# mees/hulc2

Hardware: AMD Instinct MI355X
Metric: play-sequences/sec/node (seq_len=32, 200x200 RGB) (higher is better)
Workload: dtype bf16; 1 GPU; BASELINE configs[1]: synthetic CALVIN-shaped batch, Hulc2.training_step fwd+bwd+allreduce+Adam, static CNN 200x200 + gripper CNN 84x84, lang = random (B,384) embeddings, dropout 0.1, gripper_control on; sequences_per_gpu_step=64, seq_len=32, parallelism=dp1, launch=hipGraph replay (fwd+bwd graph, all-reduce, optimizer graph), frames=fp32 NCHW, already transformed (the reference's dataloader output), gradient_allreduce=none (one rank, no process group), exact_forward_sites=encfc,goal,head,txl

## Files before the change

hulc2_amd/csrc/conv_wgrad_band.hip:

```cpp
#include "hulc_common.h"
#include "hulc_abi_internal.h"
#include "u8_frames.h"
#include <stdlib.h>

namespace {

struct WBandP {
    const void* X; const void* dY;
    int x_dtype, dy_dtype;
    int Nimg, H, W, OH, OW, R, F;
    long x_sn, x_sy, x_sx, x_sc;
    long dy_sn, dy_sy, dy_sx;
    float* partial_w;
    float* partial_b;
    int u8, pad; const int* shift; const int* fidx;
};

template <int C, int CT, int TH, int TW, int S, bool NCHW, int XCH, int YCH, int BPC, bool PURE16, bool STAMP = false>
__global__ __launch_bounds__(512, 2 * BPC) void conv_wgrad_band_kernel(WBandP p, unsigned long long* stamps = nullptr) {
    constexpr int NT = 512;
    constexpr int COUT = CT * 32;
    constexpr int K = TH * TW * C, KTN = K / 32;
    constexpr int MAXT = (KTN + 7) / 8;
    constexpr int PS = NCHW ? 2 : C * 2 + 16;
    extern __shared__ __attribute__((aligned(16))) char smem[];

    const int tid = threadIdx.x, lane = tid & 63, wave = tid >> 6;
    const int r = lane & 31, h = lane >> 5;
    const int Wb = p.W;
    const int Wp = Wb;
    const int bands = (p.OH + p.R - 1) / p.R;
    const float inv_OW = fast_rcp(p.OW);
    const int nunits = p.F > 1 ? (p.Nimg + p.F - 1) / p.F : p.Nimg * bands;
    const int rows_max = (p.F - 1) * p.H + (p.R - 1) * S + TH;
    const int npix_max = (p.F * p.R * p.OW + 15) / 16 * 16;
    constexpr bool TR = !NCHW && PURE16;
    constexpr int DROW = COUT * 2 + 16;
    const int AT_ROW = TR ? 0 : npix_max * 2 + 16;
    char* xband = smem;
    const int PP = (rows_max * Wp + 7) / 8 * 8;
    const int xbytes = NCHW ? C * PP * 2 : rows_max * Wb * PS;
    char* at = smem + (xbytes + 15) / 16 * 16;
    int* pixoff = (int*)(at + (TR ? npix_max * DROW : COUT * AT_ROW));

    constexpr bool SPLIT18 = KTN == 18 && CT == 2;
    int koff[MAXT]; bool kt_live[MAXT];
    int kts[MAXT];
    bool ct_live[MAXT][CT];
#pragma unroll
    for (int t = 0; t < MAXT; ++t) {
        int kt = wave + 8 * t;
        if (SPLIT18) kt = t < 2 ? 2 * wave + t : 16 + (wave >> 1);
        kts[t] = kt;
        kt_live[t] = SPLIT18 ? (t < 2 || wave < 4) : kt < KTN;
#pragma unroll
        for (int i = 0; i < CT; ++i) ct_live[t][i] = kt_live[t] && (!SPLIT18 || t < 2 || i == (wave & 1));
        const int k = (kt_live[t] ? kt : 0) * 32 + r;
        if (NCHW) { const int c = k / (TH * TW), kh = (k / TW) % TH, kw = k % TW; koff[t] = (c * PP + kh * Wp + kw) * 2; }
// ... 77 lines not shown
            const int qc = inb ? q : 0;
            const long off = (long)n * p.dy_sn + (long)r0 * p.dy_sy + (long)qc * p.dy_sx + ycc * 8;
            uint4 v;
            const float keep = inb ? 1.f : 0.f;
            if (PURE16 || p.dy_dtype == HULC_BF16) {
                v = *(const uint4*)((const uint16_t*)p.dY + off);
            } else {
                const float4* qq = (const float4*)((const float*)p.dY + off);
                const float4 a = qq[0], b = qq[1];
                v.x = pack_bf16x2(a.x, a.y); v.y = pack_bf16x2(a.z, a.w); v.z = pack_bf16x2(b.x, b.y); v.w = pack_bf16x2(b.z, b.w);
                bsum[0] += keep * a.x; bsum[1] += keep * a.y; bsum[2] += keep * a.z; bsum[3] += keep * a.w;
                bsum[4] += keep * b.x; bsum[5] += keep * b.y; bsum[6] += keep * b.z; bsum[7] += keep * b.w;
            }
            ypre[j] = v;
        }
    };
    int po_R = -1, po_npix = -1;
    auto stage_store = [&](int unit) {
        int n, r0, R, rows, npix; unit_geom(unit, n, r0, R, rows, npix);
        if (NCHW) {
            const int nflt = rows * p.W, items = (nflt + 7) / 8;
#pragma unroll
            for (int j = 0; j < XCH; ++j) {
                const int c = j / (XCH / C), id = tid + (j % (XCH / C)) * NT;
                if (id < items) *(uint4*)(xband + (c * PP + id * 8) * 2) = xpre[j];
            }
        } else {
            const int npx = rows * Wb, cc = tid % XCPP;
#pragma unroll
            for (int j = 0; j < XCH; ++j) {
                const int px = tid / XCPP + j * (NT / XCPP);
                if (px < npx) *(uint4*)(xband + px * PS + cc * 16) = xpre[j];
            }
        }
        const int npad = (npix + 15) / 16 * 16, ycc = tid % YCPP;
#pragma unroll
        for (int j = 0; j < YCH; ++j) {
            const int q = tid / YCPP + j * (NT / YCPP);
            if (q < npad) {
                const bool inb = q < npix;
                const uint32_t w[4] = {inb ? ypre[j].x : 0u, inb ? ypre[j].y : 0u, inb ? ypre[j].z : 0u, inb ? ypre[j].w : 0u};
                if (PURE16 || p.dy_dtype == HULC_BF16) {
#pragma unroll
                    for (int e = 0; e < 4; ++e) { bsum[2 * e] += __uint_as_float(w[e] << 16); bsum[2 * e + 1] += __uint_as_float(w[e] & 0xffff0000u); }
                }
                if (TR) *(uint4*)(at + q * DROW + ycc * 16) = make_uint4(w[0], w[1], w[2], w[3]);
                else
#pragma unroll
                for (int e = 0; e < 8; ++e) {
                    const uint16_t bits = (uint16_t)((e & 1) ? (w[e >> 1] >> 16) : (w[e >> 1] & 0xffffu));
                    *(uint16_t*)(at + (ycc * 8 + e) * AT_ROW + q * 2) = bits;
                }
            }
        }
        if (R != po_R || npix != po_npix)
        for (int q = tid; q < npad; q += NT) {
            const int qc = q < npix ? q : npix - 1;
            const int ppf = R * p.OW, f = fast_div(qc, fast_rcp(ppf)), qq = qc - f * ppf;
            const int oy = fast_div(qq, inv_OW), ox = qq - oy * p.OW;
            pixoff[q] = NCHW ? ((oy * S) * Wp + ox * S) * 2 : ((f * p.H + oy * S) * Wb + ox * S) * PS;
        }
        po_R = R; po_npix = npix;
    };

    int unit = blockIdx.x;
    if (unit < nunits) { stage_load(unit); stage_store(unit); }
    __syncthreads();
    unsigned long long t_ph[6] = {0, 0, 0, 0, 0, 0}, t_units = 0, c0 = 0, c1 = 0, c2 = 0, c3 = 0, c4 = 0, c5 = 0;
    for (; unit < nunits; unit += gridDim.x) {
        const int next = unit + gridDim.x;
        if (STAMP) c0 = __builtin_readcyclecounter();
        const bool pre = next < nunits, stagger = TR;
        int n, r0, R, rows, npix; unit_geom(unit, n, r0, R, rows, npix);
        const int nsteps = (npix + 15) / 16;
        const int bat = stagger ? ((wave * nsteps) >> 3) & ~1 : 0;
        if (pre && !stagger) stage_load(next);
        if (STAMP) c1 = __builtin_readcyclecounter();

        if (TR) {
            typedef short v4s __attribute__((ext_vector_type(4)));
// ... 90 lines not shown
            for (int t = 0; t < MAXT; ++t) {
                if (!kt_live[t]) continue;
                union { uint32_t w[4]; bf16x8_t b; } x;
#pragma unroll
                for (int e = 0; e < 4; ++e) {
                    const uint32_t lo = *(const uint16_t*)(xband + po[2 * e] + koff[t]);
                    const uint32_t hi = *(const uint16_t*)(xband + po[2 * e + 1] + koff[t]);
                    x.w[e] = lo | (hi << 16);
                }
#pragma unroll
                for (int i = 0; i < CT; ++i)
                    if (ct_live[t][i]) acc[t][i] = __builtin_amdgcn_mfma_f32_32x32x16_bf16(a[i], x.b, acc[t][i], 0, 0, 0);
            }
        }
        if (STAMP) c2 = __builtin_readcyclecounter();
        __syncthreads();
        if (STAMP) { c3 = __builtin_readcyclecounter(); asm volatile("s_waitcnt vmcnt(0)" ::: "memory"); c4 = __builtin_readcyclecounter(); }
        if (next < nunits) stage_store(next);
        if (STAMP) c5 = __builtin_readcyclecounter();
        __syncthreads();
        if (STAMP) {
            const unsigned long long c6 = __builtin_readcyclecounter();
            t_ph[0] += c1 - c0; t_ph[1] += c2 - c1; t_ph[2] += c3 - c2; t_ph[3] += c4 - c3; t_ph[4] += c5 - c4; t_ph[5] += c6 - c5; t_units += 1;
        }
    }
    if (STAMP && stamps && lane == 0) {
        unsigned long long* o = stamps + ((long)blockIdx.x * 8 + wave) * 7;
#pragma unroll
        for (int e = 0; e < 6; ++e) o[e] = t_ph[e];
        o[6] = t_units;
// ... 401 lines not shown
        static bool stamp_attr = false;
        if (!stamp_attr) {
            if (hipFuncSetAttribute((const void*)conv1_wgrad_kernel<XCH, YCH, false, true>, hipFuncAttributeMaxDynamicSharedMemorySize, 80 * 1024) != hipSuccess) return -2;
            stamp_attr = true;
        }
        conv1_wgrad_kernel<XCH, YCH, false, true><<<grid, 512, (size_t)lds_of(R), s>>>(p, (unsigned long long*)strtoull(se, nullptr, 0));
    } else
    if (p.u8) conv1_wgrad_kernel<XCH, YCH, true><<<grid, 512, (size_t)lds_of(R), s>>>(p);
    else conv1_wgrad_kernel<XCH, YCH, false><<<grid, 512, (size_t)lds_of(R), s>>>(p);
    const long Rw = 32L * K;
    const int nbw = (int)((Rw + 63) / 64);
    wband_reduce_kernel<<<nbw + (db ? 1 : 0), 1024, 0, s>>>(p.partial_w, dw, grid, Rw, accumulate, 0, 64, nbw, p.partial_b, db, 32);
    return 0;
}

template <int C, int CT, int TH, int TW, int S, bool NCHW, int XCH, int YCH, int BPC, bool PURE16 = false>
int launch_wband(WBandP& p, float* dw, float* db, void* ws, long ws_bytes, int dw_oihw, int accumulate, hipStream_t s) {
    constexpr int COUT = CT * 32, K = TH * TW * C;
    constexpr int PS = NCHW ? 2 : C * 2 + 16;
    const int Wb = p.W, Wp = Wb;
    if (NCHW && p.W % 4) return -1;
    static_assert(!NCHW || XCH % C == 0, "NCHW staging: XCH items split evenly over the channel planes");
    auto lds_of = [&](int R, int F) -> long {
        const int rows = (F - 1) * p.H + (R - 1) * S + TH;
        const long xb = NCHW ? (long)C * (((long)rows * Wp + 7) / 8 * 8) * 2 : (long)rows * Wb * PS;
        const long npad = ((long)F * R * p.OW + 15) / 16 * 16;
        const long dyb = (!NCHW && PURE16) ? npad * (COUT * 2 + 16) : (long)COUT * (npad * 2 + 16);
        return (xb + 15) / 16 * 16 + dyb + npad * 4 + 64;
    };
    auto fits = [&](int R, int F) -> bool {
        const int rows = (F - 1) * p.H + (R - 1) * S + TH;
        const long xitems = NCHW ? ((long)rows * p.W + 7) / 8 * C : (long)rows * Wb * (C / 8);
        const long yitems = (((long)F * R * p.OW + 15) / 16 * 16) * (COUT / 8);
        return lds_of(R, F) <= (160 * 1024 - 256) / BPC && xitems <= (long)XCH * 512 && yitems <= (long)YCH * 512;
    };
    int R = p.OH, F = 1;
    while (R > 1 && !fits(R, 1)) --R;
    if (!fits(R, 1)) return -1;
    int nunits;
    if (R == p.OH && !NCHW) {
        while (F < p.Nimg && fits(R, F + 1)) ++F;
        nunits = (p.Nimg + F - 1) / F;
    } else {
        const int bands = (p.OH + R - 1) / R;
        R = (p.OH + bands - 1) / bands;
        nunits = p.Nimg * bands;
    }
    if ((long)F * R * p.OW < 96) return -1;
    p.R = R; p.F = F;
    const int slots = 256 * BPC;
    const int per = (nunits + slots - 1) / slots;
    const int grid = (nunits + per - 1) / per;
    if ((long)grid * COUT * (K + 1) * 4 > ws_bytes) return -1;
    p.partial_w = (float*)ws;
    p.partial_b = db ? p.partial_w + (long)grid * COUT * K : nullptr;
    auto kern = conv_wgrad_band_kernel<C, CT, TH, TW, S, NCHW, XCH, YCH, BPC, PURE16>;
    static bool attr_set = false;
    if (!attr_set) {
        if (hipFuncSetAttribute((const void*)kern, hipFuncAttributeMaxDynamicSharedMemorySize, 160 * 1024) != hipSuccess) return -2;
        attr_set = true;
    }
    const char* se = getenv("HULC_WB_STAMPS");
    if (se && *se && PURE16 && !NCHW) {
        auto kst = conv_wgrad_band_kernel<C, CT, TH, TW, S, NCHW, XCH, YCH, BPC, PURE16, true>;
        static bool st_attr = false;
        if (!st_attr) {
            if (hipFuncSetAttribute((const void*)kst, hipFuncAttributeMaxDynamicSharedMemorySize, 160 * 1024) != hipSuccess) return -2;
            st_attr = true;
        }
        kst<<<grid, 512, (size_t)lds_of(R, F), s>>>(p, (unsigned long long*)strtoull(se, nullptr, 0));
    } else
    kern<<<grid, 512, (size_t)lds_of(R, F), s>>>(p, nullptr);
    const long Rw = (long)COUT * K;
    const int nbw = (int)((Rw + 63) / 64);
    wband_reduce_kernel<<<nbw + (db ? 1 : 0), 1024, 0, s>>>(p.partial_w, dw, grid, Rw, accumulate, (dw_oihw && !NCHW) ? C : 0, TH * TW, nbw, p.partial_b, db,
                                                          COUT);
    return 0;
}
// ... 33 lines not shown
            q.xs = (const void* const*)x_slot; q.xs2 = (const void* const*)x2_slot;
            if ((x_slot || x2_slot) && (u8 || !x_slot || (x2_slot && !x2) || ((uintptr_t)x_slot | (uintptr_t)x2_slot) % 8))
                return hulc_fail(-6, "conv1 weight gradient: frame slots are for fp32 frames (x_slot with every launch, x2_slot next to x2), 8-byte aligned");
            if (x2) {
                q.X2 = u8 ? (const float*)((const unsigned char*)x2 - (long)n_split * 3 * H * W) : (const float*)x2 - (long)n_split * 3 * H * W;
                q.nsplit = n_split;
            }
            rc = launch_conv1_wgrad(q, dw, db, ws, ws_bytes, accumulate, s);
        }
    }
    else return (x2 || x_slot) ? hulc_fail(-6, "conv weight gradient: x2 / frame slots are for conv1 only") : 1;
    if (rc == -1) return 1;
    if (rc < 0) return hulc_fail(-8, "conv wgrad band: could not raise the dynamic LDS limit");
    return 0;
}
```

hulc2_amd/csrc/pointwise.hip:

```cpp
#include "hulc_common.h"
#include "hulc_abi_internal.h"
#include <stdlib.h>

namespace {

__global__ __launch_bounds__(256) void spatial_softmax_fwd_kernel(const void* __restrict__ x, int x_dtype, int N, int HW, int C,
                                                                  const float* __restrict__ xmap, const float* __restrict__ ymap,
                                                                  const float* __restrict__ temperature, float* __restrict__ out,
                                                                  float* __restrict__ stats) {
    __shared__ float red[4][4][64];
    const int lane = threadIdx.x & 63, wave = threadIdx.x >> 6;
    const int n = blockIdx.x;
    const bool act = lane < C;
    const float invT = 1.0f / temperature[0];
    const long base = (long)n * HW * C + lane;
    const int per = (HW + 3) / 4, p0 = wave * per, p1 = p0 + per < HW ? p0 + per : HW;
    float m = -INFINITY;
    if (act)
        for (int p = p0; p < p1; ++p) m = fmaxf(m, load_elem(x, x_dtype, base + (long)p * C) * invT);
    red[wave][0][lane] = m;
    __syncthreads();
    m = fmaxf(fmaxf(red[0][0][lane], red[1][0][lane]), fmaxf(red[2][0][lane], red[3][0][lane]));
    float s = 0.f, sx = 0.f, sy = 0.f;
    if (act)
// ... 162 lines not shown
}
__global__ __launch_bounds__(256) void spatial_softmax_bwd64_kernel(const void* __restrict__ x, int x_dtype, int HW,
                                                                    const float* __restrict__ xmap, const float* __restrict__ ymap,
                                                                    const float* __restrict__ temperature, const float* __restrict__ out,
                                                                    const float* __restrict__ stats, const float* __restrict__ dout,
                                                                    void* __restrict__ dx, int dx_dtype, int relu_mask) {
    const int lane = threadIdx.x & 63, wave = threadIdx.x >> 6;
    const int cg = lane & 7, pl = lane >> 3;
    const int n = blockIdx.x;
    const float invT = 1.0f / temperature[0];
    const long base = (long)n * HW * 64 + cg * 8;
    float m[8], k[8], ex[8], ey[8], gx[8], gy[8];
#pragma unroll
    for (int j = 0; j < 8; ++j) {
        const int c = cg * 8 + j;
        m[j] = stats[((long)n * 64 + c) * 2]; k[j] = invT / stats[((long)n * 64 + c) * 2 + 1];
        ex[j] = out[(long)n * 128 + 2 * c]; ey[j] = out[(long)n * 128 + 2 * c + 1];
        gx[j] = dout[(long)n * 128 + 2 * c]; gy[j] = dout[(long)n * 128 + 2 * c + 1];
    }
    for (int p = wave * 8 + pl; p < HW; p += 32) {
        Chunk8 c; chunk_load_contig(c, x, x_dtype, base + (long)p * 64);
        const float xm = xmap[p], ym = ymap[p];
        float g[8];
#pragma unroll
        for (int j = 0; j < 8; ++j) {
            g[j] = k[j] * __expf(c.v[j] * invT - m[j]) * (gx[j] * (xm - ex[j]) + gy[j] * (ym - ey[j]));
            if (relu_mask && !(c.v[j] > 0.f)) g[j] = 0.f;
        }
        const long o = base + (long)p * 64;
        if (dx_dtype == HULC_BF16) *(uint4*)((uint16_t*)dx + o) = make_uint4(pack_bf16x2(g[0], g[1]), pack_bf16x2(g[2], g[3]), pack_bf16x2(g[4], g[5]), pack_bf16x2(g[6], g[7]));
        else { ((float4*)((float*)dx + o))[0] = make_float4(g[0], g[1], g[2], g[3]); ((float4*)((float*)dx + o))[1] = make_float4(g[4], g[5], g[6], g[7]); }
    }
}


__global__ __launch_bounds__(256) void layernorm_fwd_kernel(const float* __restrict__ x, const float* __restrict__ o, float drop_p,
                                                            unsigned long long seed, const unsigned long long* __restrict__ seed_dev,
                                                            const float* __restrict__ gamma,
                                                            const float* __restrict__ beta, float eps, int R, int D,
                                                            float* __restrict__ pre_out, float* __restrict__ y,
                                                            float* __restrict__ mean_out, float* __restrict__ rstd_out,
                                                            int n_o = 1, long o_stride = 0, long ld_y = 0) {
    const int lane = threadIdx.x & 63;
// ... 649 lines not shown
```

hulc2_amd/functional.py:

```python
from typing import List, Optional, Sequence, Tuple

import os

import torch

from . import gradsink
from . import kernels as kn
from .shadow import weight_operand


def _scoped(cls):
    fwd, bwd = cls.forward, cls.backward

    def forward(ctx, *args):
        ctx._compute = kn.backward_compute()
        return fwd(ctx, *args)

    def backward(ctx, *grads):
        if ctx._compute == kn.get_compute():
            return bwd(ctx, *grads)
        with kn.compute_scope(ctx._compute):
            return bwd(ctx, *grads)

    forward.__doc__, backward.__doc__ = fwd.__doc__, bwd.__doc__
# ... 329 lines not shown
    def forward(ctx, grad_premasked, aug, w1, b1, w2, b2, w3, b3, *xs):
        xs = [_c(x) for x in xs]
        pad, shifts, indices = (aug if aug is not None else (0, [None] * len(xs), [None] * len(xs)))
        Ns = [x.shape[0] if ix is None else ix.numel() for x, ix in zip(xs, indices)]
        N = sum(Ns)
        u8 = xs[0].dtype == torch.uint8
        if u8:
            _, H, W, C = xs[0].shape
        else:
            _, C, H, W = xs[0].shape
        ws, bs = (w1, w2, w3), (b1, b2, b3)
        acts, dims = [], []
        inp, h, w_, cin = None, H, W, C
        want_bits = _act_dtype() == torch.bfloat16 and any(ctx.needs_input_grad[2:8])
        bits = [None, None, None]
        exact_out = False
        if isinstance(grad_premasked, tuple):
            grad_premasked, exact_out = grad_premasked
        a3_exact = _act_dtype() == torch.bfloat16 and kn.base_mode() == "bf16" and (exact_out or "a3" in kn.fp32_sites())
        for li, (k, s) in enumerate(ConvStackFn.GEOM):
            cout = ws[li].shape[0]
            nchw = li == 0
            w2d = weight_operand(ws[li], "oihw_flat" if nchw else "ohwi")
            oh, ow = kn.conv_out_hw(h, w_, k, k, s)
            twin = a3_exact and li == 2
            f16_twin = twin and (h, w_, cin, cout, k, s) == (23, 23, 64, 64, 3, 1)
            y = torch.empty(N, oh, ow, cout, dtype=(torch.float16 if f16_twin else torch.float32) if twin else _act_dtype(), device=xs[0].device)
            y16 = torch.empty(N, oh, ow, cout, dtype=torch.bfloat16, device=xs[0].device) if twin else None
            if want_bits and li < 2 and cout % 32 == 0 and (li > 0 or cout == 32):
                bits[li] = torch.empty(N * oh * ow * (cout // 32), dtype=torch.int32, device=xs[0].device)
            if li == 0:
                off = 0
                w_lo = weight_operand(ws[0], "oihw_flat_lo") if (not u8 and _act_dtype() == torch.bfloat16 and kn.base_mode() == "bf16"
# ... 24 lines not shown
                        raise
                    y = torch.empty(N, oh, ow, cout, dtype=torch.float32, device=xs[0].device)
                    kn.conv2d_fwd(inp, w2d, bs[li], y, N, h, w_, cin, cout, k, k, s, nchw, relu=True, relu_bits=bits[li], y_bf16=y16)
            dims.append((h, w_, cin, cout, k, s, nchw))
            acts.append(y16 if y16 is not None else y)
            inp, h, w_, cin = y, oh, ow, cout
        a3_f32 = y if (a3_exact and y16 is not None) else None
        saved = acts
        if kn.backward_compute() == "bf16" and acts[0].dtype != torch.bfloat16:
            saved = []
            for a in acts:
                h = torch.empty(a.shape, dtype=torch.bfloat16, device=a.device)
                kn.cast_f32_to_bf16(a, h, a.numel())
                saved.append(h)
        ctx.g_dtype = saved[1].dtype
        ctx.save_for_backward(saved[0], saved[1], saved[2], w2, w3, *xs)
        ctx.conv_w, ctx.conv_b = ws, bs
        ctx.relu_bits = bits
        ctx.aug = (pad, shifts, indices)
        ctx.meta = (dims, grad_premasked, Ns)
        if a3_f32 is not None:
            ctx.mark_non_differentiable(a3_f32)
            ctx.set_materialize_grads(False)
            return acts[2], a3_f32
        return acts[2]

    @staticmethod
    def backward(ctx, da3, *unused):
        a1, a2, a3, w2, w3, *xs = ctx.saved_tensors
        dims, premasked, Ns = ctx.meta
        if da3 is None:
            da3 = torch.zeros_like(a3)
        N = sum(Ns)
        g = _c(da3)
        if premasked and g.dtype != ctx.g_dtype:
            h = torch.empty(g.shape, dtype=ctx.g_dtype, device=g.device)
            kn.cast_f32_to_bf16(g, h, g.numel())
            g = h
        if not premasked:
            gz = torch.empty(g.shape, dtype=torch.float32, device=g.device)
            kn.relu_bwd(g.float() if g.dtype != torch.float32 else g, a3, gz, g.numel())
            g = gz
        inputs = (None, a1, a2)
        weights = (None, w2, w3)
        grads_w, grads_b = [None] * 3, [None] * 3
# ... 13 lines not shown
                paired = False
                if _conv1_pair_ok(xs, xs[0].dtype == torch.uint8, None, cout, shifts, indices) and g.dtype == torch.bfloat16:
                    pair_shift, pair_index = getattr(ctx, "pair_aug", (None, None))
                    try:
                        kn.conv2d_bwd_weight(xs[0], g, dw, db, N, h, w_, cin, cout, k, k, s, nchw, dw_oihw=True, accumulate=acc,
                                             x2=None if pair_index is not None else xs[1], aug_shift=pair_shift, aug_pad=pad, frame_index=pair_index)
                        paired = True
                    except kn._L.HulcKernelError as e:
                        if not _pair_not_covered(e):
                            raise
                if not paired:
                    for j, (x, n, sh, ix) in enumerate(zip(xs, Ns, shifts, indices)):
                        kn.conv2d_bwd_weight(x, g[off:off + n], dw, db, n, h, w_, cin, cout, k, k, s, nchw, dw_oihw=True, accumulate=acc or j > 0,
                                             aug_shift=sh, aug_pad=pad, frame_index=ix)
                        off += n
            else:
                kn.conv2d_bwd_weight(inputs[li], g, dw, db, N, h, w_, cin, cout, k, k, s, nchw, dw_oihw=True, accumulate=acc)
            grads_w[li] = None if sunk else dw.view(cout, cin, k, k)
            grads_b[li] = None if sunk else db
            if li > 0:
                inp = inputs[li]
                wt = weight_operand(weights[li], "ihwo")
                dx = torch.empty(N, h, w_, cin, dtype=inp.dtype, device=g.device)
                kn.conv2d_bwd_data(g, wt, dx, inp, N, h, w_, cin, cout, k, k, s, relu_bits=ctx.relu_bits[li - 1])
                g = dx
        return (None, None, grads_w[0], grads_b[0], grads_w[1], grads_b[1], grads_w[2], grads_b[2], *([None] * len(xs)))


def conv_stack(x, params, grad_premasked=False, aug_pad=0, aug_shifts=None, frame_index=None, exact_out=False):
    xs = list(x) if isinstance(x, (list, tuple)) else [x]
    aug = None
    if xs[0].dtype == torch.uint8:
        sh = list(aug_shifts) if isinstance(aug_shifts, (list, tuple)) else [aug_shifts] * len(xs)
        ix = list(frame_index) if isinstance(frame_index, (list, tuple)) else [frame_index] * len(xs)
        aug = (int(aug_pad), [None if t is None else _c(t.reshape(-1, 2).to(torch.int32)) for t in sh],
               [None if t is None else _c(t.reshape(-1).to(torch.int32)) for t in ix])
    out = ConvStackFn.apply((bool(grad_premasked), True) if exact_out else grad_premasked, aug, *params, *xs)
    if isinstance(out, tuple):
        out[0]._hulc_f32 = out[1]
        return out[0]
    return out


def exact_map(a: torch.Tensor):
    t = getattr(a, "_hulc_f32", None)
    return t if (t is not None and t.shape == a.shape) else None


@_scoped
class SpatialSoftmaxFn(torch.autograd.Function):

    @staticmethod
    def forward(ctx, a, xmap, ymap, temperature, a_exact=None):
        N, H, W, C = a.shape
        out = _f32(N, 2 * C, like=a)
# ... 909 lines not shown
```

hulc2_amd/kernels.py:

```python
import ctypes

import torch

from . import lib as _L

F32, BF16, F16 = 0, 1, 2
_COMPUTE = {"bf16": BF16, "fp32": F32, "f32": F32}
_compute_mode = BF16


_base_mode = "bf16"
_bwd_mode = None


def set_compute(mode: str) -> None:
    global _compute_mode, _base_mode, _bwd_mode
    if mode not in ("bf16", "fp32", "mixed"):
        raise ValueError(mode)
    _base_mode, _bwd_mode = mode, None
    _compute_mode = _COMPUTE["bf16" if mode == "mixed" else mode]


def get_compute() -> str:
    return "bf16" if _compute_mode == BF16 else "fp32"
# ... 440 lines not shown
                      aug_shift=None, aug_pad=0, frame_index=None, x2=None):
    _require_cuda(x, dy, dw, db)
    _require_contiguous(x=x, dy=dy, dw=dw)
    d = _conv_desc(N, H, W, Cin, Cout, KH, KW, stride, x_nchw, F32 if x.dtype == torch.uint8 else _dt(x), _dt(dy), F32, False, compute)
    d.dw_oihw, d.dw_accumulate = int(dw_oihw), int(accumulate)
    _u8_frames(d, x, aug_shift, aug_pad, frame_index)
    _second_frames(d, x, x2, N, Cin, H, W)
    if compute is None and frame_index is None and dy.dtype == torch.bfloat16:
        _slot_fields(d, x, x2, H, W, Cin, Cout, KH, stride, x_nchw)
    nbytes = _L.load().hulc_conv2d_bwd_weight_workspace(ctypes.byref(d))
    ws = torch.empty(nbytes // 4, dtype=torch.float32, device=x.device)
    oh, ow = conv_out_hw(H, W, KH, KW, stride)
    macs = float(N) * oh * ow * Cout * Cin * KH * KW
    _call("hulc_conv2d_bwd_weight", ctypes.byref(d), x, dy, dw, db, ws, key=("conv2d_bwd_weight", N, H, W, Cin, Cout, KH, stride), flops=2 * macs,
          nbytes=_nbytes(x, dy, dw, db) + (_nbytes(x2) if x2 is not None else 0))
    return dw, db


_c = ctypes


def _call(name, *args, key=None, flops=0.0, nbytes=0.0):
    lib = _L.load()
    conv = []
    for a in args:
        if isinstance(a, torch.Tensor):
            _require_cuda(a)
            a = a.data_ptr()
        conv.append(a)
    with _Timed(key or (name,), flops, nbytes):
# ... 970 lines not shown
```

hulc2_amd/models/perceptual_encoders/vision_network.py:

```python
from typing import Optional, Tuple

import torch
import torch.nn as nn

from hulc2_amd import functional as HF
from hulc2_amd import kernels as kn


class SpatialSoftmax(nn.Module):

    def __init__(self, num_rows: int, num_cols: int, temperature: Optional[float] = None):
        super().__init__()
        self.num_rows, self.num_cols = num_rows, num_cols
        a = torch.linspace(-1.0, 1.0, num_cols).reshape(-1, 1).expand(num_cols, num_rows)
        b = torch.linspace(-1.0, 1.0, num_rows).reshape(1, -1).expand(num_cols, num_rows)
        self.register_buffer("x_map", a.reshape(-1).clone())
        self.register_buffer("y_map", b.reshape(-1).clone())
        if temperature:
            self.register_buffer("temperature", torch.ones(1) * temperature)
        else:
            self.temperature = nn.Parameter(torch.ones(1))
        self.coords = None

    def forward(self, a_nhwc: torch.Tensor) -> torch.Tensor:
        if isinstance(self.temperature, nn.Parameter) and self.temperature.requires_grad:
            raise NotImplementedError("learnable spatial-softmax temperature is not on the configured path "
                                      "(conf/model/perceptual_encoder/rgb_static/default.yaml: spatial_softmax_temp 1.0)")
        out = HF.spatial_softmax(a_nhwc, self.x_map, self.y_map, self.temperature)
        self.coords = out.detach()
        return out


class VisionNetwork(nn.Module):
    def __init__(self, input_width: int, input_height: int, activation_function: str, dropout_vis_fc: float,
                 l2_normalize_output: bool, visual_features: int, num_c: int, use_sinusoid: bool,
                 spatial_softmax_temp: float):
        super().__init__()
        if activation_function != "ReLU" or use_sinusoid or l2_normalize_output or dropout_vis_fc != 0.0:
            raise NotImplementedError("hulc2_amd VisionNetwork implements the configured path only: ReLU, no sinusoid, "
                                      "no l2-normalise, dropout_vis_fc 0 (conf/model/perceptual_encoder/rgb_static/default.yaml)")
        self.act_fn = nn.ReLU()
        w, h = input_width, input_height
        for k, s in ((8, 4), (4, 2), (3, 1)):
# ... 2 lines not shown
        self.spatial_softmax = SpatialSoftmax(num_rows=w, num_cols=h, temperature=temp)
        self.conv_model = nn.Sequential(nn.Conv2d(num_c, 32, 8, stride=4), self.act_fn, nn.Conv2d(32, 64, 4, stride=2),
                                        self.act_fn, nn.Conv2d(64, 64, 3, stride=1), self.act_fn)
        self.fc1 = nn.Sequential(nn.Linear(128, 512), self.act_fn, nn.Dropout(dropout_vis_fc))
        self.fc2 = nn.Linear(512, visual_features)
        self.ln = nn.LayerNorm(visual_features)

    def lo_operands(self):
        return [(self.fc1[0].weight, "lo"), (self.fc2.weight, "lo"), (self.conv_model[0].weight, "oihw_flat_lo")]

    def conv_params(self):
        c = self.conv_model
        return (c[0].weight, c[0].bias, c[2].weight, c[2].bias, c[4].weight, c[4].bias)

    def forward(self, x: torch.Tensor, aug_shift=None, aug_pad: int = 0, frame_index=None, pre_ln: bool = False) -> torch.Tensor:
        a3 = HF.conv_stack(x, self.conv_params(), grad_premasked=True, aug_pad=aug_pad, aug_shifts=aug_shift, frame_index=frame_index)
        feat = self.spatial_softmax(a3)
        with kn.site_scope("encfc"):
            y = HF.mlp2_rows(feat, self.fc1[0].weight, self.fc1[0].bias, self.fc2.weight, self.fc2.bias)
        if pre_ln:
            return y
        return HF.layer_norm(y, self.ln.weight, self.ln.bias, self.ln.eps)

    @staticmethod
    def calc_out_size(w: int, h: int, kernel_size: int, padding: int, stride: int) -> Tuple[int, int]:
        return (w - kernel_size + 2 * padding) // stride + 1, (h - kernel_size + 2 * padding) // stride + 1
```

include/hulc2_amd.h:

```cpp
#ifndef HULC2_AMD_H
#define HULC2_AMD_H

#ifdef __cplusplus
extern "C" {
#endif

#define HULC_F32 0
#define HULC_BF16 1
#define HULC_F16 2

const char* hulc_last_error(void);
int hulc_abi_version(void);
int hulc_set_coop_share(int n);
int hulc_stream_create(void** out);

typedef struct {
    const void* A; const void* B; void* C;
    const float* bias; const void* add; const void* mask;
    int M, N, K;
    long lda, ldb, ldc, ld_add, ld_mask;
    int a_dtype, b_dtype, c_dtype, add_dtype, mask_dtype;
    int a_kmajor, b_kmajor;
    int relu, accumulate;
    float alpha, mask_scale, drop_p;
// ... 18 lines not shown
    int aug_pad;
    const int* aug_shift;
    const int* frame_index;
    void* relu_bits;
    const void* w_lo;
    const void* x2;
    int n_split;
    const void* x_slot;
    const void* x2_slot;
    void* y_bf16;
} hulc_conv_desc;
int hulc_conv2d_fwd(const hulc_conv_desc* d, const void* x, const void* w, const float* bias, void* y, void* stream);
int hulc_conv2d_bwd_data(const hulc_conv_desc* d, const void* dy, const void* wt, void* dx, const void* relu_src, void* stream);
long hulc_conv2d_bwd_weight_workspace(const hulc_conv_desc* d);
int hulc_conv2d_bwd_weight(const hulc_conv_desc* d, const void* x, const void* dy, float* dw, float* db, void* ws, void* stream);

int hulc_spatial_softmax_fwd(const void* x, int x_dtype, int N, int HW, int C, const float* xmap, const float* ymap,
                             const float* temperature, float* out, float* stats, void* stream);
int hulc_spatial_softmax_bwd(const void* x, int x_dtype, int N, int HW, int C, const float* xmap, const float* ymap,
                             const float* temperature, const float* out, const float* stats, const float* dout,
                             void* dx, int dx_dtype, int relu_mask, void* stream);
int hulc_layernorm_fwd(const float* x, const float* o, float drop_p, unsigned long long seed, const unsigned long long* seed_dev,
                       const float* gamma, const float* beta, float eps, int R, int D, float* pre_out, float* y, float* mean,
                       float* rstd, void* stream);
int hulc_layernorm_slab_fwd(const float* x, const float* o, int n_o, long o_stride, float drop_p, unsigned long long seed,
                            const unsigned long long* seed_dev, const float* gamma, const float* beta, float eps, int R, int D,
                            float* pre_out, float* y, float* mean, float* rstd, void* stream);
int hulc_layernorm_fwd_ld(const float* x, const float* gamma, const float* beta, float eps, int R, int D, float* y, long ld_y, float* mean,
                          float* rstd, void* stream);
int hulc_layernorm_bwd_ld(const float* dy, long ld_dy, const float* pre, const float* mean, const float* rstd, const float* gamma, int R, int D,
// ... 261 lines not shown
```

Measured before the change: 21030 play-sequences/s.

## Fuse spatial-softmax backward into conv3 weight-gradient band kernel

Moves the spatial-softmax forward inside the conv stack autograd function. Its backward, which turns a3 plus the softmax stats into dA3, now runs in the staging phase of the 64->64 conv3 weight-gradient band kernel. The kernel computes dA3 per tile in registers, writes it out for the later data-gradient pass, and uses it straight away for dW/db. This removes a separate pointwise kernel and one read of dA3 from memory, at the cost of extra LDS for the coordinate maps and stats, extra waitcnt syncs, and a geometry-specific path with a fallback.

```diff
diff --git a/hulc2_amd/csrc/conv_wgrad_band.hip b/hulc2_amd/csrc/conv_wgrad_band.hip
--- a/hulc2_amd/csrc/conv_wgrad_band.hip
+++ b/hulc2_amd/csrc/conv_wgrad_band.hip
@@ -1,6 +1,7 @@
 #include "hulc_common.h"
 #include "hulc_abi_internal.h"
 #include "u8_frames.h"
+#include "spatial_softmax.h"
 #include <stdlib.h>
 
 namespace {
@@ -14,9 +15,12 @@
     float* partial_w;
     float* partial_b;
     int u8, pad; const int* shift; const int* fidx;
+    const float* xmap; const float* ymap; const float* temperature;
+    const float* ss_out; const float* ss_stats; const float* ss_dout;
+    void* dy_out;
 };
 
-template <int C, int CT, int TH, int TW, int S, bool NCHW, int XCH, int YCH, int BPC, bool PURE16, bool STAMP = false>
+template <int C, int CT, int TH, int TW, int S, bool NCHW, int XCH, int YCH, int BPC, bool PURE16, bool STAMP = false, bool SSM = false>
 __global__ __launch_bounds__(512, 2 * BPC) void conv_wgrad_band_kernel(WBandP p, unsigned long long* stamps = nullptr) {
     constexpr int NT = 512;
     constexpr int COUT = CT * 32;
@@ -42,6 +46,12 @@
     const int xbytes = NCHW ? C * PP * 2 : rows_max * Wb * PS;
     char* at = smem + (xbytes + 15) / 16 * 16;
     int* pixoff = (int*)(at + (TR ? npix_max * DROW : COUT * AT_ROW));
+    static_assert(!SSM || (TR && COUT == 64), "the fused spatial-softmax backward is built for the bf16 64-channel NHWC instance");
+    constexpr int SSM_HWP = 448;
+    float* const ssc = (float*)(pixoff + npix_max);
+    float* const smx = ssc + 384;
+    float* const smy = smx + SSM_HWP;
+    const float ss_invT = SSM ? 1.0f / p.temperature[0] : 1.f;
 
     constexpr bool SPLIT18 = KTN == 18 && CT == 2;
     int koff[MAXT]; bool kt_live[MAXT];
@@ -149,6 +159,14 @@
             }
             ypre[j] = v;
         }
+        if (SSM && wave == 0) {
+            const long so = (long)n * 128 + (lane & 31) * 4;
+            __builtin_amdgcn_global_load_lds((const void __attribute__((address_space(1)))*)((lane < 32 ? p.ss_stats : p.ss_out) + so),
+                                             (void __attribute__((address_space(3)))*)ssc, 16, 0, 0);
+            if (lane < 32)
+                __builtin_amdgcn_global_load_lds((const void __attribute__((address_space(1)))*)(p.ss_dout + so),
+                                                 (void __attribute__((address_space(3)))*)(ssc + 256), 16, 0, 0);
+        }
     };
     int po_R = -1, po_npix = -1;
     auto stage_store = [&](int unit) {
@@ -169,12 +187,42 @@
             }
         }
         const int npad = (npix + 15) / 16 * 16, ycc = tid % YCPP;
+        if (SSM) {
+            uint32_t yw[YCH][4];
+            float xm[YCH], ym[YCH];
+#pragma unroll
+            for (int j = 0; j < YCH; ++j) {
+                const int q = tid / YCPP + j * (NT / YCPP);
+                const int pos = r0 * p.OW + (q < npix ? q : 0);
+                xm[j] = smx[pos]; ym[j] = smy[pos];
+                yw[j][0] = ypre[j].x; yw[j][1] = ypre[j].y; yw[j][2] = ypre[j].z; yw[j][3] = ypre[j].w;
+            }
+#pragma unroll
+            for (int e = 0; e < 4; ++e) {
+                const float4 st = *(const float4*)(ssc + ycc * 16 + 4 * e), eo = *(const float4*)(ssc + 128 + ycc * 16 + 4 * e),
+                             go = *(const float4*)(ssc + 256 + ycc * 16 + 4 * e);
+                const float k0 = hulc_ssm::bwd_scale(ss_invT, st.y), k1 = hulc_ssm::bwd_scale(ss_invT, st.w);
+#pragma unroll
+                for (int j = 0; j < YCH; ++j) {
+                    const float a0 = __uint_as_float(yw[j][e] << 16), a1 = __uint_as_float(yw[j][e] & 0xffff0000u);
+                    yw[j][e] = pack_bf16x2(hulc_ssm::bwd_elem(a0, ss_invT, st.x, k0, go.x, go.y, eo.x, eo.y, xm[j], ym[j], true),
+                                           hulc_ssm::bwd_elem(a1, ss_invT, st.z, k1, go.z, go.w, eo.z, eo.w, xm[j], ym[j], true));
+                    asm volatile("" : "+v"(yw[j][e]));
+                }
+            }
+#pragma unroll
+            for (int j = 0; j < YCH; ++j) ypre[j] = make_uint4(yw[j][0], yw[j][1], yw[j][2], yw[j][3]);
+        }
 #pragma unroll
         for (int j = 0; j < YCH; ++j) {
             const int q = tid / YCPP + j * (NT / YCPP);
             if (q < npad) {
                 const bool inb = q < npix;
                 const uint32_t w[4] = {inb ? ypre[j].x : 0u, inb ? ypre[j].y : 0u, inb ? ypre[j].z : 0u, inb ? ypre[j].w : 0u};
+                if (SSM) {
+                    if (inb)
+                        *(uint4*)((uint16_t*)p.dy_out + ((long)n * p.dy_sn + (long)r0 * p.dy_sy + (long)q * p.dy_sx + ycc * 8)) = make_uint4(w[0], w[1], w[2], w[3]);
+                }
                 if (PURE16 || p.dy_dtype == HULC_BF16) {
 #pragma unroll
                     for (int e = 0; e < 4; ++e) { bsum[2 * e] += __uint_as_float(w[e] << 16); bsum[2 * e + 1] += __uint_as_float(w[e] & 0xffff0000u); }
@@ -199,6 +247,13 @@
     };
 
     int unit = blockIdx.x;
+    if (SSM) {
+        for (int i = tid; i < p.OH * p.OW; i += NT) { smx[i] = p.xmap[i]; smy[i] = p.ymap[i]; }
+        if (unit < nunits) stage_load(unit);
+        __builtin_amdgcn_s_waitcnt(0x0F70);
+        __syncthreads();
+        if (unit < nunits) stage_store(unit);
+    } else
     if (unit < nunits) { stage_load(unit); stage_store(unit); }
     __syncthreads();
     unsigned long long t_ph[6] = {0, 0, 0, 0, 0, 0}, t_units = 0, c0 = 0, c1 = 0, c2 = 0, c3 = 0, c4 = 0, c5 = 0;
@@ -319,6 +374,7 @@
             }
         }
         if (STAMP) c2 = __builtin_readcyclecounter();
+        if (SSM && wave == 0) __builtin_amdgcn_s_waitcnt(0x0F70);
         __syncthreads();
         if (STAMP) { c3 = __builtin_readcyclecounter(); asm volatile("s_waitcnt vmcnt(0)" ::: "memory"); c4 = __builtin_readcyclecounter(); }
         if (next < nunits) stage_store(next);
@@ -750,7 +806,7 @@
     return 0;
 }
 
-template <int C, int CT, int TH, int TW, int S, bool NCHW, int XCH, int YCH, int BPC, bool PURE16 = false>
+template <int C, int CT, int TH, int TW, int S, bool NCHW, int XCH, int YCH, int BPC, bool PURE16 = false, bool SSM = false>
 int launch_wband(WBandP& p, float* dw, float* db, void* ws, long ws_bytes, int dw_oihw, int accumulate, hipStream_t s) {
     constexpr int COUT = CT * 32, K = TH * TW * C;
     constexpr int PS = NCHW ? 2 : C * 2 + 16;
@@ -762,7 +818,7 @@
         const long xb = NCHW ? (long)C * (((long)rows * Wp + 7) / 8 * 8) * 2 : (long)rows * Wb * PS;
         const long npad = ((long)F * R * p.OW + 15) / 16 * 16;
         const long dyb = (!NCHW && PURE16) ? npad * (COUT * 2 + 16) : (long)COUT * (npad * 2 + 16);
-        return (xb + 15) / 16 * 16 + dyb + npad * 4 + 64;
+        return (xb + 15) / 16 * 16 + dyb + npad * 4 + 64 + (SSM ? (384 + 2 * 448) * 4 : 0);
     };
     auto fits = [&](int R, int F) -> bool {
         const int rows = (F - 1) * p.H + (R - 1) * S + TH;
@@ -783,6 +839,7 @@
         nunits = p.Nimg * bands;
     }
     if ((long)F * R * p.OW < 96) return -1;
+    if (SSM && (F != 1 || p.OH * p.OW > 448)) return -1;
     p.R = R; p.F = F;
     const int slots = 256 * BPC;
     const int per = (nunits + slots - 1) / slots;
@@ -790,14 +847,14 @@
     if ((long)grid * COUT * (K + 1) * 4 > ws_bytes) return -1;
     p.partial_w = (float*)ws;
     p.partial_b = db ? p.partial_w + (long)grid * COUT * K : nullptr;
-    auto kern = conv_wgrad_band_kernel<C, CT, TH, TW, S, NCHW, XCH, YCH, BPC, PURE16>;
+    auto kern = conv_wgrad_band_kernel<C, CT, TH, TW, S, NCHW, XCH, YCH, BPC, PURE16, false, SSM>;
     static bool attr_set = false;
     if (!attr_set) {
         if (hipFuncSetAttribute((const void*)kern, hipFuncAttributeMaxDynamicSharedMemorySize, 160 * 1024) != hipSuccess) return -2;
         attr_set = true;
     }
     const char* se = getenv("HULC_WB_STAMPS");
-    if (se && *se && PURE16 && !NCHW) {
+    if (se && *se && PURE16 && !NCHW && !SSM) {
         auto kst = conv_wgrad_band_kernel<C, CT, TH, TW, S, NCHW, XCH, YCH, BPC, PURE16, true>;
         static bool st_attr = false;
         if (!st_attr) {
@@ -861,3 +918,30 @@
     if (rc < 0) return hulc_fail(-8, "conv wgrad band: could not raise the dynamic LDS limit");
     return 0;
 }
+
+extern "C" int hulc_conv2d_bwd_weight_ssm(const hulc_conv_desc* d, const void* x, const void* a3, const float* xmap, const float* ymap,
+                                          const float* temperature, const float* out, const float* stats, const float* dout, void* dy_out,
+                                          float* dw, float* db, void* ws, void* stream) {
+    if (!d || !x || !a3 || !xmap || !ymap || !temperature || !out || !stats || !dout || !dy_out || !dw || !ws)
+        return hulc_fail(-1, "hulc_conv2d_bwd_weight_ssm: null pointer");
+    if (d->N <= 0 || d->x_nchw || d->Cin != 64 || d->Cout != 64 || d->KH != 3 || d->KW != 3 || d->stride != 1 || d->H != 23 || d->W != 23)
+        return hulc_fail(-2, "hulc_conv2d_bwd_weight_ssm: covers the 64 -> 64 channel 3 x 3 stride-1 layer on 23 x 23 NHWC frames only");
+    if (d->x_dtype != HULC_BF16 || d->y_dtype != HULC_BF16 || d->compute != HULC_BF16)
+        return hulc_fail(-6, "hulc_conv2d_bwd_weight_ssm: bf16 maps and bf16 compute only");
+    if (d->x2 || d->x_slot || d->x2_slot || d->x_u8_nhwc || d->frame_index || d->aug_shift)
+        return hulc_fail(-6, "hulc_conv2d_bwd_weight_ssm: a second frame tensor, frame slots and uint8 frames belong to conv1");
+    if (((uintptr_t)x | (uintptr_t)a3 | (uintptr_t)dy_out | (uintptr_t)out | (uintptr_t)stats | (uintptr_t)dout) % 16)
+        return hulc_fail(-4, "hulc_conv2d_bwd_weight_ssm: x, a3, dy_out, out, stats and dout are 16-byte aligned");
+    WBandP p;
+    p.u8 = 0; p.pad = 0; p.shift = nullptr; p.fidx = nullptr;
+    p.X = x; p.dY = a3; p.x_dtype = HULC_BF16; p.dy_dtype = HULC_BF16;
+    p.Nimg = d->N; p.H = 23; p.W = 23; p.OH = 21; p.OW = 21; p.R = 1; p.F = 1;
+    p.x_sn = 23L * 23 * 64; p.x_sy = 23L * 64; p.x_sx = 64; p.x_sc = 1;
+    p.dy_sn = 21L * 21 * 64; p.dy_sy = 21L * 64; p.dy_sx = 64;
+    p.xmap = xmap; p.ymap = ymap; p.temperature = temperature; p.ss_out = out; p.ss_stats = stats; p.ss_dout = dout; p.dy_out = dy_out;
+    const int rc = launch_wband<64, 2, 3, 3, 1, false, 5, 4, 1, true, true>(p, dw, db, ws, hulc_conv2d_bwd_weight_workspace(d), d->dw_oihw, d->dw_accumulate,
+                                                                           (hipStream_t)stream);
+    if (rc == -1) return hulc_fail(-6, "hulc_conv2d_bwd_weight_ssm: the band plan does not fit (LDS or workspace)");
+    if (rc < 0) return hulc_fail(-8, "conv wgrad band: could not raise the dynamic LDS limit");
+    return hulc_check_launch("hulc_conv2d_bwd_weight_ssm");
+}
diff --git a/hulc2_amd/csrc/pointwise.hip b/hulc2_amd/csrc/pointwise.hip
--- a/hulc2_amd/csrc/pointwise.hip
+++ b/hulc2_amd/csrc/pointwise.hip
@@ -1,5 +1,6 @@
 #include "hulc_common.h"
 #include "hulc_abi_internal.h"
+#include "spatial_softmax.h"
 #include <stdlib.h>
 
 namespace {
@@ -200,7 +201,7 @@
 #pragma unroll
     for (int j = 0; j < 8; ++j) {
         const int c = cg * 8 + j;
-        m[j] = stats[((long)n * 64 + c) * 2]; k[j] = invT / stats[((long)n * 64 + c) * 2 + 1];
+        m[j] = stats[((long)n * 64 + c) * 2]; k[j] = hulc_ssm::bwd_scale(invT, stats[((long)n * 64 + c) * 2 + 1]);
         ex[j] = out[(long)n * 128 + 2 * c]; ey[j] = out[(long)n * 128 + 2 * c + 1];
         gx[j] = dout[(long)n * 128 + 2 * c]; gy[j] = dout[(long)n * 128 + 2 * c + 1];
     }
@@ -209,10 +210,7 @@
         const float xm = xmap[p], ym = ymap[p];
         float g[8];
 #pragma unroll
-        for (int j = 0; j < 8; ++j) {
-            g[j] = k[j] * __expf(c.v[j] * invT - m[j]) * (gx[j] * (xm - ex[j]) + gy[j] * (ym - ey[j]));
-            if (relu_mask && !(c.v[j] > 0.f)) g[j] = 0.f;
-        }
+        for (int j = 0; j < 8; ++j) g[j] = hulc_ssm::bwd_elem(c.v[j], invT, m[j], k[j], gx[j], gy[j], ex[j], ey[j], xm, ym, relu_mask != 0);
         const long o = base + (long)p * 64;
         if (dx_dtype == HULC_BF16) *(uint4*)((uint16_t*)dx + o) = make_uint4(pack_bf16x2(g[0], g[1]), pack_bf16x2(g[2], g[3]), pack_bf16x2(g[4], g[5]), pack_bf16x2(g[6], g[7]));
         else { ((float4*)((float*)dx + o))[0] = make_float4(g[0], g[1], g[2], g[3]); ((float4*)((float*)dx + o))[1] = make_float4(g[4], g[5], g[6], g[7]); }
diff --git a/hulc2_amd/csrc/spatial_softmax.h b/hulc2_amd/csrc/spatial_softmax.h
--- /dev/null
+++ b/hulc2_amd/csrc/spatial_softmax.h
@@ -0,0 +1,14 @@
+#pragma once
+#include "hulc_common.h"
+
+namespace hulc_ssm {
+
+HULC_DEVICE float bwd_scale(float invT, float sum) { return invT / sum; }
+
+HULC_DEVICE float bwd_elem(float x, float invT, float m, float k, float gx, float gy, float ex, float ey, float xm, float ym, bool relu_mask) {
+    float g = k * __expf(x * invT - m) * (gx * (xm - ex) + gy * (ym - ey));
+    if (relu_mask && !(x > 0.f)) g = 0.f;
+    return g;
+}
+
+}
diff --git a/hulc2_amd/functional.py b/hulc2_amd/functional.py
--- a/hulc2_amd/functional.py
+++ b/hulc2_amd/functional.py
@@ -367,9 +367,9 @@
         inp, h, w_, cin = None, H, W, C
         want_bits = _act_dtype() == torch.bfloat16 and any(ctx.needs_input_grad[2:8])
         bits = [None, None, None]
-        exact_out = False
+        exact_out, ssm = False, None
         if isinstance(grad_premasked, tuple):
-            grad_premasked, exact_out = grad_premasked
+            grad_premasked, exact_out, ssm = (*grad_premasked, None)[:3]
         a3_exact = _act_dtype() == torch.bfloat16 and kn.base_mode() == "bf16" and (exact_out or "a3" in kn.fp32_sites())
         for li, (k, s) in enumerate(ConvStackFn.GEOM):
             cout = ws[li].shape[0]
@@ -424,11 +424,20 @@
                 kn.cast_f32_to_bf16(a, h, a.numel())
                 saved.append(h)
         ctx.g_dtype = saved[1].dtype
-        ctx.save_for_backward(saved[0], saved[1], saved[2], w2, w3, *xs)
         ctx.conv_w, ctx.conv_b = ws, bs
         ctx.relu_bits = bits
         ctx.aug = (pad, shifts, indices)
         ctx.meta = (dims, grad_premasked, Ns)
+        ctx.ssm = False
+        if ssm is not None and a3_f32 is None and saved is acts and kn.backward_compute() == "bf16" and kn.get_compute() == "bf16" \
+                and kn.conv3_ssm_covered(acts[1], acts[2], N, *dims[2][:4], dims[2][4], dims[2][4], dims[2][5]):
+            xmap, ymap, temperature = ssm
+            out, stats = _f32(N, 2 * dims[2][3], like=acts[2]), _f32(N, dims[2][3], 2, like=acts[2])
+            kn.spatial_softmax_fwd(acts[2], N, acts[2].shape[1] * acts[2].shape[2], dims[2][3], xmap, ymap, temperature, out, stats)
+            ctx.save_for_backward(saved[0], saved[1], saved[2], w2, w3, *xs, xmap, ymap, temperature, out, stats)
+            ctx.ssm = True
+            return out
+        ctx.save_for_backward(saved[0], saved[1], saved[2], w2, w3, *xs)
         if a3_f32 is not None:
             ctx.mark_non_differentiable(a3_f32)
             ctx.set_materialize_grads(False)
@@ -439,6 +448,11 @@
     def backward(ctx, da3, *unused):
         a1, a2, a3, w2, w3, *xs = ctx.saved_tensors
         dims, premasked, Ns = ctx.meta
+        ssm = None
+        if ctx.ssm:
+            *xs, xmap, ymap, temperature, ss_out, ss_stats = xs
+            ssm = (xmap, ymap, temperature, ss_out, ss_stats, _c(da3))
+            da3, premasked = a3, True
         if da3 is None:
             da3 = torch.zeros_like(a3)
         N = sum(Ns)
@@ -482,6 +496,15 @@
                         kn.conv2d_bwd_weight(x, g[off:off + n], dw, db, n, h, w_, cin, cout, k, k, s, nchw, dw_oihw=True, accumulate=acc or j > 0,
                                              aug_shift=sh, aug_pad=pad, frame_index=ix)
                         off += n
+            elif li == 2 and ssm is not None:
+                xmap, ymap, temperature, ss_out, ss_stats, dout = ssm
+                g = torch.empty_like(a3)
+                try:
+                    kn.conv2d_bwd_weight_ssm(a2, a3, xmap, ymap, temperature, ss_out, ss_stats, dout, g, dw, db, N, h, w_, cin, cout, k, k, s,
+                                             dw_oihw=True, accumulate=acc)
+                except kn._L.HulcKernelError:
+                    kn.spatial_softmax_bwd(a3, N, a3.shape[1] * a3.shape[2], cout, xmap, ymap, temperature, ss_out, ss_stats, dout, g, relu_mask=True)
+                    kn.conv2d_bwd_weight(a2, g, dw, db, N, h, w_, cin, cout, k, k, s, nchw, dw_oihw=True, accumulate=acc)
             else:
                 kn.conv2d_bwd_weight(inputs[li], g, dw, db, N, h, w_, cin, cout, k, k, s, nchw, dw_oihw=True, accumulate=acc)
             grads_w[li] = None if sunk else dw.view(cout, cin, k, k)
@@ -495,7 +518,7 @@
         return (None, None, grads_w[0], grads_b[0], grads_w[1], grads_b[1], grads_w[2], grads_b[2], *([None] * len(xs)))
 
 
-def conv_stack(x, params, grad_premasked=False, aug_pad=0, aug_shifts=None, frame_index=None, exact_out=False):
+def conv_stack(x, params, grad_premasked=False, aug_pad=0, aug_shifts=None, frame_index=None, exact_out=False, ssm=None):
     xs = list(x) if isinstance(x, (list, tuple)) else [x]
     aug = None
     if xs[0].dtype == torch.uint8:
@@ -503,10 +526,13 @@
         ix = list(frame_index) if isinstance(frame_index, (list, tuple)) else [frame_index] * len(xs)
         aug = (int(aug_pad), [None if t is None else _c(t.reshape(-1, 2).to(torch.int32)) for t in sh],
                [None if t is None else _c(t.reshape(-1).to(torch.int32)) for t in ix])
-    out = ConvStackFn.apply((bool(grad_premasked), True) if exact_out else grad_premasked, aug, *params, *xs)
+    mode = (bool(grad_premasked), bool(exact_out), tuple(ssm)) if ssm is not None else (bool(grad_premasked), True) if exact_out else grad_premasked
+    out = ConvStackFn.apply(mode, aug, *params, *xs)
     if isinstance(out, tuple):
         out[0]._hulc_f32 = out[1]
-        return out[0]
+        out = out[0]
+    if ssm is not None and out.dim() == 4:
+        return spatial_softmax(out, *ssm)
     return out
 
 
diff --git a/hulc2_amd/kernels.py b/hulc2_amd/kernels.py
--- a/hulc2_amd/kernels.py
+++ b/hulc2_amd/kernels.py
@@ -478,6 +478,27 @@
     macs = float(N) * oh * ow * Cout * Cin * KH * KW
     _call("hulc_conv2d_bwd_weight", ctypes.byref(d), x, dy, dw, db, ws, key=("conv2d_bwd_weight", N, H, W, Cin, Cout, KH, stride), flops=2 * macs,
           nbytes=_nbytes(x, dy, dw, db) + (_nbytes(x2) if x2 is not None else 0))
+    return dw, db
+
+
+def conv3_ssm_covered(x, a3, N, H, W, Cin, Cout, KH, KW, stride, compute=None) -> bool:
+    return ((H, W, Cin, Cout, KH, KW, stride) == (23, 23, 64, 64, 3, 3, 1) and N > 0 and x.dtype == torch.bfloat16 and a3.dtype == torch.bfloat16
+            and x.is_contiguous() and a3.is_contiguous() and x.data_ptr() % 16 == 0 and a3.data_ptr() % 16 == 0
+            and (_compute_mode if compute is None else compute) == BF16)
+
+
+def conv2d_bwd_weight_ssm(x, a3, xmap, ymap, temperature, out, stats, dout, dy_out, dw, db, N, H, W, Cin, Cout, KH, KW, stride,
+                          compute=None, dw_oihw=False, accumulate=False):
+    _require_cuda(x, a3, xmap, ymap, temperature, out, stats, dout, dy_out, dw, db)
+    _require_contiguous(x=x, a3=a3, out=out, stats=stats, dout=dout, dy_out=dy_out, dw=dw)
+    d = _conv_desc(N, H, W, Cin, Cout, KH, KW, stride, False, _dt(x), _dt(a3), F32, False, compute)
+    d.dw_oihw, d.dw_accumulate = int(dw_oihw), int(accumulate)
+    nbytes = _L.load().hulc_conv2d_bwd_weight_workspace(ctypes.byref(d))
+    ws = torch.empty(nbytes // 4, dtype=torch.float32, device=x.device)
+    oh, ow = conv_out_hw(H, W, KH, KW, stride)
+    macs = float(N) * oh * ow * Cout * Cin * KH * KW
+    _call("hulc_conv2d_bwd_weight_ssm", ctypes.byref(d), x, a3, xmap, ymap, temperature, out, stats, dout, dy_out, dw, db, ws,
+          key=("conv2d_bwd_weight_ssm", N, H, W, Cin, Cout, KH, stride), flops=2 * macs, nbytes=_nbytes(x, a3, dy_out, dw, db))
     return dw, db
 
 
diff --git a/hulc2_amd/models/perceptual_encoders/vision_network.py b/hulc2_amd/models/perceptual_encoders/vision_network.py
--- a/hulc2_amd/models/perceptual_encoders/vision_network.py
+++ b/hulc2_amd/models/perceptual_encoders/vision_network.py
@@ -22,11 +22,20 @@
             self.temperature = nn.Parameter(torch.ones(1))
         self.coords = None
 
-    def forward(self, a_nhwc: torch.Tensor) -> torch.Tensor:
+    def check_temperature(self) -> None:
         if isinstance(self.temperature, nn.Parameter) and self.temperature.requires_grad:
             raise NotImplementedError("learnable spatial-softmax temperature is not on the configured path "
                                       "(conf/model/perceptual_encoder/rgb_static/default.yaml: spatial_softmax_temp 1.0)")
+
+    def forward(self, a_nhwc: torch.Tensor) -> torch.Tensor:
+        self.check_temperature()
         out = HF.spatial_softmax(a_nhwc, self.x_map, self.y_map, self.temperature)
+        self.coords = out.detach()
+        return out
+
+    def behind(self, conv_stack) -> torch.Tensor:
+        self.check_temperature()
+        out = conv_stack((self.x_map, self.y_map, self.temperature))
         self.coords = out.detach()
         return out
 
@@ -59,8 +68,8 @@
         return (c[0].weight, c[0].bias, c[2].weight, c[2].bias, c[4].weight, c[4].bias)
 
     def forward(self, x: torch.Tensor, aug_shift=None, aug_pad: int = 0, frame_index=None, pre_ln: bool = False) -> torch.Tensor:
-        a3 = HF.conv_stack(x, self.conv_params(), grad_premasked=True, aug_pad=aug_pad, aug_shifts=aug_shift, frame_index=frame_index)
-        feat = self.spatial_softmax(a3)
+        feat = self.spatial_softmax.behind(lambda ssm: HF.conv_stack(x, self.conv_params(), grad_premasked=True, aug_pad=aug_pad, aug_shifts=aug_shift,
+                                                                     frame_index=frame_index, ssm=ssm))
         with kn.site_scope("encfc"):
             y = HF.mlp2_rows(feat, self.fc1[0].weight, self.fc1[0].bias, self.fc2.weight, self.fc2.bias)
         if pre_ln:
diff --git a/include/hulc2_amd.h b/include/hulc2_amd.h
--- a/include/hulc2_amd.h
+++ b/include/hulc2_amd.h
@@ -56,6 +56,9 @@
 int hulc_conv2d_bwd_data(const hulc_conv_desc* d, const void* dy, const void* wt, void* dx, const void* relu_src, void* stream);
 long hulc_conv2d_bwd_weight_workspace(const hulc_conv_desc* d);
 int hulc_conv2d_bwd_weight(const hulc_conv_desc* d, const void* x, const void* dy, float* dw, float* db, void* ws, void* stream);
+int hulc_conv2d_bwd_weight_ssm(const hulc_conv_desc* d, const void* x, const void* a3, const float* xmap, const float* ymap,
+                               const float* temperature, const float* out, const float* stats, const float* dout, void* dy_out,
+                               float* dw, float* db, void* ws, void* stream);
 
 int hulc_spatial_softmax_fwd(const void* x, int x_dtype, int N, int HW, int C, const float* xmap, const float* ymap,
                              const float* temperature, float* out, float* stats, void* stream);
```

Result: no change. 21030 play-sequences/s, median of 2 (+0.0%).
